# haoyu94/RoITr

Measured on AMD Instinct MI355X. Metric: point-cloud pairs/s, higher is better.
Workload: dtype f32; 1 GPU; 3DMatch-sized synthetic pairs: 5000 pts/cloud src+tgt, fp32, 3DMatch test settings (P=256 patches x 64 pts, 100 Sinkhorn iterations), full RIGA_v2 forward; n_points=5000, weights=closed-form, variant 'selective' (roitr_amd/weights.py); normals: field, cloud=uniform, correspondences_found=66241517

## Files before the change

### include/roitr_engine.h

```cpp
#ifndef ROITR_ENGINE_H
#define ROITR_ENGINE_H

#include <stddef.h>

#ifdef __cplusplus
extern "C" {
#endif

#ifndef ROITR_POINTOPS_H
typedef struct ihipStream_t* roitr_stream_t;
#endif

typedef struct RoitrGemm {
    int M, N, K;
    const float* A; const float* A2; int lda; const int* a_idx; int a_limit;
    const float* W; int ldw; const int* w_idx; int w_limit;
    const float* bias; float alpha; int relu;
    float* C; int ldc;
    int batch; long sA, sW, sC, sBias, sAidx, sWidx;
    const int* seg_off; int seg_a0, seg_w0;
    const float* ln_gamma; const float* ln_beta; const float* ln_res; const int* ln_res_idx; const float* ln_post;
    int ln_relu; float ln_eps;
    int bf16;
    const float* A_cat; int lda_cat; int k_cat;
    const float* ip_feat; const int* ip_idx; const float* ip_dist2;
    const int* a_cat_idx;
    const int* batch_live;
    long w_piece;
} RoitrGemm;
#define ROITR_BF16_W 1
#define ROITR_BF16_A 2
#define ROITR_BF16_C 4
#define ROITR_BF16_X3 8
int roitr_gemm(const RoitrGemm* g, roitr_stream_t stream);
int roitr_gemm_bf16_supported(const RoitrGemm* g);
int roitr_f32_to_bf16(long n, const float* src, unsigned short* dst, roitr_stream_t stream);
int roitr_gemm_x3_supported(const RoitrGemm* g);
int roitr_split_bf16x3(long n, const float* src, unsigned short* dst, long piece, roitr_stream_t stream);

int roitr_add_layernorm(int M, int C, const float* x, const float* res, const int* res_idx, const float* gamma,
                        const float* beta, const float* post_add, int relu, float eps, float* out, roitr_stream_t stream);
int roitr_add_layernorm_interp(int M, int C, const float* x, const float* res, const int* res_idx, const float* gamma,
                               const float* beta, int relu, float eps, const float* ip_feat, const int* ip_idx, const float* ip_dist2,
                               float* out, roitr_stream_t stream);
int roitr_l2_normalize(int M, int C, const float* x, float* out, roitr_stream_t stream);
int roitr_transpose(int rows, int cols, const float* in, int ld_in, float* out, int ld_out, roitr_stream_t stream);
int roitr_add_vectors(int n, const float* a, const float* b, float* out, roitr_stream_t stream);
int roitr_interp3_add(int n, int C, const float* feat, const int* idx, const float* dist2, const float* base, float* out,
                      roitr_stream_t stream);
int roitr_segment_mean(int b, int C, const float* x, const int* offset, float* out, roitr_stream_t stream);
int roitr_sinusoid(long rows, int C, const float* vals, const float* div_term, float* out, roitr_stream_t stream);
int roitr_geo_embed(long rows, int C, int angle_k, const float* d_idx, const float* a_idx, const float* div_term,
                    const float* Wd, const float* bd, const float* Wa, const float* ba, float* out, roitr_stream_t stream);
int roitr_split3_bf16(long n, const float* src, unsigned short* dst, roitr_stream_t stream);
int roitr_geo_embed_split(long rows, int C, int angle_k, const float* d_idx, const float* a_idx, const float* div_term,
                          const unsigned short* Wd3, const float* bd, const unsigned short* Wa3, const float* ba, float* out,
                          roitr_stream_t stream);
int roitr_geo_embed_bf16(long rows, int C, int angle_k, const float* d_idx, const float* a_idx, const float* div_term,
                         const unsigned short* Wd, const float* bd, const unsigned short* Wa, const float* ba, float* out,
                         roitr_stream_t stream);
int roitr_geo_embed_bf16_out(long rows, int C, int angle_k, const float* d_idx, const float* a_idx, const float* div_term,
                             const unsigned short* Wd, const float* bd, const unsigned short* Wa, const float* ba,
                             unsigned short* out, roitr_stream_t stream);
size_t roitr_geo_table_floats(int C, int n_int_d, int n_int_a);
int roitr_geo_table_build(int C, const float* div_term, const float* Wd, const float* bd, const float* Wa, const float* ba,
                          float interval, int n_int_d, int n_int_a, float* table, double* fit);
int roitr_geo_embed_table(long rows, int C, int angle_k, const float* d_idx, const float* a_idx, const float* table, float interval,
                          int n_int_d, int n_int_a, const float* div_term, const float* Wd, const float* bd, const float* Wa,
                          const float* ba, void* out, int out_bf16, roitr_stream_t stream);
int roitr_geo_combine(long rows, int C, int k, const float* pd, const float* pa, float* out, roitr_stream_t stream);
int roitr_gather_rows(long rows, int C, const float* in, const int* idx, int limit, float* out, roitr_stream_t stream);
int roitr_compose_idx(int n, const int* outer, const int* inner, int* out, roitr_stream_t stream);
int roitr_calc_ppf(int m, int k, const float* centre_xyz, const float* centre_normals, const float* ref_xyz,
                   const float* ref_normals, const int* group_idx, float* out, roitr_stream_t stream);

typedef struct RoitrLocalAttn {
    int M, K, H, heads;
    const float* q; int ldq;
    const float* k; int ldk;
    const float* v; int ldv;
    const int* group_idx; const float* ppf;
    const float* wvpe; const float* bvpe;
    float scale;
    float* out; int ldo;
    const void* node_order;
    int bf16;
    const float* wpe; const float* bpe;
} RoitrLocalAttn;
// ... 154 lines not shown
    int num_corr;
    int point_limit;
    int fine_topk, fine_mutual, fine_use_global_score;
    float fine_conf;
    int n_geo_layers;
    int geo_is_cross[16];
    float matching_radius;
    int adaptive_coarse;
    float occlusion_radius;
    int operand_dtype;
} RoitrEngineConfig;

typedef struct RoitrForwardIO {
    int pairs;
    const int* n_points;
    const float* points_geom;
    const float* normals;
    const float* feats;
    const float* points_out;
    const float* rot;
    const float* trans;
    float* node_xyz;
    float* node_feats;
    float* point_feats;
    int* node_masks;
    int* node_knn_idx;
    int* node_knn_mask;
    int* tgt_corr; int* src_corr; float* corr_scores; int* n_corr;
    float* tgt_knn_pts; float* src_knn_pts;
    int* tgt_knn_masks; int* src_knn_masks;
    float* matching_scores;
    float* out_tgt_pts; float* out_src_pts; float* out_scores; int* out_patch;
    int* fine_offsets;
    int* n_out;
    float* gt_node_occ;
    int* gt_corr_idx;
    float* gt_corr_overlaps;
    int* gt_corr_count;
    void* inputs_ready;
    int* patch_offsets;
    int* pair_starts;
    int patch_slots;
} RoitrForwardIO;

void* roitr_engine_create(const RoitrEngineConfig* cfg);
void roitr_engine_destroy(void* engine);
int roitr_engine_set_param(void* engine, const char* name, const float* device_ptr, long numel);
int roitr_engine_finalize(void* engine, roitr_stream_t stream);
int roitr_engine_geo_table_info(void* engine, double* info);
int roitr_engine_forward(void* engine, const RoitrForwardIO* io, roitr_stream_t stream);
int roitr_engine_forward_graph(void* engine, const RoitrForwardIO* io, roitr_stream_t stream);
int roitr_engine_graph_count(void* engine);
int roitr_engine_set_phase_overlap(void* engine, int on);
int roitr_engine_scratch_info(void* engine, long* out5);
int roitr_engine_set_tap(void* engine, const char* name, void* device_ptr);
int roitr_engine_set_inject(void* engine, const char* name, const void* device_ptr);
void roitr_level_sizes(int n, int* out4);


int roitr_inlier_counts(int pairs, const int* starts, const float* src_pts, const float* tgt_pts, const float* rot,
                        const float* trans, float radius, int* inliers, roitr_stream_t stream);
int roitr_coarse_hits(int pairs, int num_corr, const int* n_corr, const int* tgt_corr, const int* src_corr, int gt_cap,
                      const int* gt_idx, const float* gt_overlaps, const int* gt_count, float acceptance_overlap, int* hits,
                      roitr_stream_t stream);


size_t roitr_registration_workspace_bytes(int pairs, int total_rows, int iterations, int chunks);
int roitr_ransac_correspondences(int pairs, const int* starts, int total_rows, const float* src_pts, const float* tgt_pts,
                                 const float* scores, const unsigned int* pair_keys, int sample_mode, int n_points, int ransac_n,
                                 float distance_threshold, float edge_similarity, int iterations, int refine_iters, int refine_weighted,
                                 unsigned long long seed, int chunks, void* workspace, size_t workspace_bytes, float* transforms,
                                 int* inliers, int* best_iteration, int* valid_hypotheses, int* n_used, int* selected,
                                 roitr_stream_t stream);
int roitr_ransac_samples(int pairs, const int* n, const unsigned int* pair_keys, unsigned long long seed, int it0, int count, int* out,
                         roitr_stream_t stream);
int roitr_weighted_procrustes(int batch, int n, const float* src_pts, const float* tgt_pts, const float* weights, float weight_thresh,
                              float eps, float* transforms, roitr_stream_t stream);


#define ROITR_LGR_NO_ROWS 1
#define ROITR_LGR_NO_LOCAL 2
#define ROITR_LGR_EMPTY_REFIT 4
size_t roitr_lgr_workspace_bytes(int pairs, int total_rows);
int roitr_lgr_batch(int pairs, const int* starts, int total_rows, const float* src_pts, const float* tgt_pts, const float* scores,
                    const int* row_patch, float radius, int min_rows, int steps, void* workspace, size_t workspace_bytes,
                    float* transforms, int* inliers, int* best_hypothesis, int* best_first_row, int* hypotheses, int* local_inliers,
                    int* status, int* hyp_starts, int* hyp_first_row, float* hyp_transforms, int* hyp_counts, roitr_stream_t stream);


#define ROITR_COMPAT_NO_ROWS 1
#define ROITR_COMPAT_NO_HYPOTHESIS 2
#define ROITR_COMPAT_EMPTY_REFIT 4
#define ROITR_COMPAT_TRUNCATED 8
size_t roitr_compat_workspace_bytes(int pairs, int total_rows, int max_rows, int max_seeds, int k);
int roitr_compat_batch(int pairs, const int* starts, int total_rows, const float* src_pts, const float* tgt_pts, const float* scores,
                       float compat_dist, float radius, int max_rows, int max_seeds, int k, int steps, void* workspace,
                       size_t workspace_bytes, float* transforms, int* inliers, int* best_rank, int* best_seed_row, int* seeds,
                       int* hypotheses, int* local_inliers, int* status, int* degree, int* seed_rows, int* seed_members,
                       float* hyp_transforms, int* hyp_counts, roitr_stream_t stream);


#define ROITR_NFMR_FEW_ANCHORS 1
#define ROITR_NFMR_NO_METRIC 2
#define ROITR_NFMR_BAD_INDEX 4
#define ROITR_NFMR_BAD_OFFSETS 8
size_t roitr_nfmr_workspace_bytes(int pairs, int total_corr, int total_metric);
// ... 39 lines not shown
```

### roitr_amd/csrc/engine.cpp

```cpp
#include <hip/hip_runtime.h>
#include <math.h>
#include <stdio.h>
#include <string.h>

#include <map>
#include <string>
#include <vector>

#include "common.h"
#include "prof.h"
#include "roitr_engine.h"
#include "roitr_pointops.h"

#define CHK(x)                    \
    do {                          \
        int s__ = (x);            \
        if (s__ != 0) return s__; \
    } while (0)

namespace {

constexpr int HEADS = 4;
constexpr int GRID_MIN_POINTS = 768;

struct Lin {
    const float* w = nullptr; const float* b = nullptr; int out = 0, in = 0;
    const unsigned short* wb = nullptr;
};

struct LocalT {
    Lin emb, in_proj, q, k, v, p, vp, lin, out_proj;
    const float* norm_w = nullptr; const float* norm_b = nullptr;
    int in_dim = 0, H = 0, out_dim = 0;
    float* wqkv = nullptr;
    unsigned short* wqkv_b = nullptr;
    float* bqkv = nullptr;
    float* wqkv_x = nullptr; float* bqkv_x = nullptr; unsigned short* wqkv_x_b = nullptr;
    float* wkT_x = nullptr;
    float* wqqt_x = nullptr; float* bqqt_x = nullptr;
    float* wcat = nullptr; float* bcat = nullptr; unsigned short* wcat_b = nullptr;
    const float* wpe = nullptr; const float* bpe = nullptr;
    float* wvpe = nullptr;
    float* bvpe = nullptr;
    const float* bn2_w = nullptr; const float* bn2_b = nullptr;
};

struct Up {
    Lin l1, l2; const float* l1n_w = nullptr; const float* l1n_b = nullptr; const float* l2n_w = nullptr; const float* l2n_b = nullptr;
};

struct Ffn {
    Lin expand, squeeze; const float* n_w = nullptr; const float* n_b = nullptr;
};

struct GeoLayer {
    bool cross = false;
    Lin q, k, v, p, vp, lin, pos_lin;
    const float *n_w = nullptr, *n_b = nullptr, *pn_w = nullptr, *pn_b = nullptr;
    Ffn out, pos;
    float* wqkv = nullptr; float* bqkv = nullptr;
    float* wpT = nullptr;
    unsigned short* wqkv_b = nullptr; unsigned short* wpT_b = nullptr;
};

struct Arena {
    char* base = nullptr; size_t cap = 0, off = 0, peak = 0;
    bool fail = false;
    template <typename T> T* get(size_t count)
    {
        const size_t bytes = (count * sizeof(T) + 255) & ~(size_t)255;
        if (off + bytes > cap) { fail = true; return (T*)base; }
        T* p = base ? (T*)(base + off) : nullptr;
        off += bytes;
        if (off > peak) peak = off;
        return p;
    }
};

struct Engine {
    RoitrEngineConfig cfg;
    std::map<std::string, std::pair<const float*, long>> params;
    std::map<std::string, void*> taps;
    std::map<std::string, const void*> injects;
    bool finalized = false;
    int planes[4];
    int nblocks[4] = {2, 3, 3, 3};
    int nsample[4] = {8, 16, 16, 16};
    LocalT enc[4][3];
    LocalT dec[4];
    Up up[4];
    Lin geo_in, geo_out, proj_d, proj_a, coarse_proj, fine_proj;
    const float* geo_div = nullptr;
    float* geo_div_own = nullptr;
    float* geo_tab = nullptr; float geo_tab_h = 0.f; int geo_tab_nd = 0, geo_tab_na = 0; double geo_tab_fit[6] = {0, 0, 0, 0, 0, 0};
    std::vector<GeoLayer> geo;
    const float* ot_alpha = nullptr;
    float* first_consts = nullptr;
    Arena warena;
    Arena arena;
    Arena barena;
    Arena garena[2];
    int gpar = 0;
    int cur_par = -1;
    hipEvent_t gend[2] = {nullptr, nullptr};
    bool gend_rec[2] = {false, false};
    bool ahead_off = false;
    bool garena_short = false;
    static constexpr int RING = 4;
    char* pinned[RING] = {nullptr, nullptr, nullptr, nullptr}; size_t pinned_cap[RING] = {0, 0, 0, 0};
    hipEvent_t pinned_ev[RING] = {nullptr, nullptr, nullptr, nullptr};
    int ring_pos = 0;
    hipStream_t side = nullptr;
    enum Ev {
        EV_MAIN_BEGIN,
        EV_LEVEL2_GEOM_DONE,
        EV_LEVEL3_GEOM_DONE,
        EV_LEVEL4_GEOM_DONE,
        EV_LEVEL1_WS_FREE,
        EV_EMBED_DONE,
        EV_NN3_DONE,
        EV_TAIL_DONE,
        EV_ERROR_JOIN,
        EV_DESC_COPIED,
        EV_LEVEL1_GROUPS_READY,
        EV_ENCODER_DONE,
        EV_BRANCH_DONE,
        EV_BRANCH_ERROR_JOIN,
        NEV
    };
    static Ev ev_level_done(int l) { return (Ev)(EV_LEVEL2_GEOM_DONE + l - 1); }
    hipEvent_t ev[NEV] = {};
    bool side_forked = false;
    hipStream_t branch = nullptr;
    int phase_overlap = 1;
    bool branch_forked = false;
    bool on_branch = false;
    std::string err;
    hipStream_t fin_stream = nullptr;
    struct GraphEntry {
        std::vector<long> key;
        hipGraph_t graph = nullptr; hipGraphExec_t exec = nullptr;
        char* pin = nullptr; size_t pin_cap = 0;
        long epoch = -1;
        bool warmed = false, failed = false;
        unsigned long stamp = 0;
    };
    std::vector<GraphEntry> graphs;
    long arena_epoch = 0;
    unsigned long graph_clock = 0;
    char* capture_pin = nullptr;
    std::map<std::pair<const float*, long>, unsigned short*> x3;
    std::vector<const float*> frag_weights;
};

thread_local Engine* g_engine = nullptr;

int use_x3(RoitrGemm& g, hipStream_t st)
{
    Engine* E = g_engine;
    if (!E || E->cfg.operand_dtype != 2 || !E->finalized || g.bf16 || g.K < 256 || g.ldw != g.K || g.batch != 1 || g.ln_gamma) return 0;
    RoitrGemm t = g;
    t.bf16 = ROITR_BF16_X3; t.w_piece = (long)g.N * g.K;
    const long numel = (long)g.N * g.K;
    const auto key = std::make_pair(g.W, numel);
    auto it = E->x3.find(key);
    unsigned short* w3 = nullptr;
    if (it != E->x3.end()) w3 = it->second;
    else {
        if (E->capture_pin) return 0;
        if (hipMalloc((void**)&w3, sizeof(unsigned short) * 3 * (size_t)numel) != hipSuccess) { (void)hipGetLastError(); return 0; }
        if (roitr_split_bf16x3(numel, g.W, w3, numel, st) != ROITR_OK) { (void)hipFree(w3); return 0; }
        E->x3[key] = w3;
    }
    t.W = reinterpret_cast<const float*>(w3);
    if (!roitr_gemm_x3_supported(&t)) return 0;
    g = t;
    return 0;
}

const float* P(Engine& E, const std::string& name, long expect)
{
    auto it = E.params.find(name);
    if (it == E.params.end()) { if (E.err.empty()) E.err = "missing parameter " + name; return nullptr; }
    if (expect > 0 && it->second.second != expect) {
        if (E.err.empty()) E.err = "parameter " + name + " has " + std::to_string(it->second.second) + " elements, expected " + std::to_string(expect);
        return nullptr;
    }
    return it->second.first;
}

Lin lin(Engine& E, const std::string& prefix, int out, int in)
{
    Lin l;
    l.w = P(E, prefix + ".weight", (long)out * in);
    l.b = P(E, prefix + ".bias", out);
    l.out = out; l.in = in;
    if (E.cfg.operand_dtype == 1 && l.w) {
        unsigned short* wb = E.warena.get<unsigned short>((size_t)out * in);
        if (!E.warena.fail && roitr_f32_to_bf16((long)out * in, l.w, wb, E.fin_stream) == 0) l.wb = wb;
    }
    return l;
}

bool bf16_layer(const unsigned short* Wb, int K) { return Wb != nullptr && K % 64 == 0; }
int use_bf16(RoitrGemm& g, const float* W, const unsigned short* Wb, int bf)
{
    if (Wb) {
        g.W = reinterpret_cast<const float*>(Wb);
        g.bf16 = ROITR_BF16_W | bf;
        if (roitr_gemm_bf16_supported(&g)) return 0;
        g.W = W; g.bf16 = 0;
    }
    if (bf) { roitr_set_error("engine: bf16-stored activation routed to an fp32 layer", __FILE__, __LINE__); return ROITR_ERR_ARG; }
    return 0;
}
int gemm(hipStream_t st, int M, int N, int K, const float* A, int lda, const float* W, int ldw, const float* bias, float* C, int ldc,
         bool relu = false, const int* a_idx = nullptr, const float* A2 = nullptr, float alpha = 1.0f, const unsigned short* Wb = nullptr,
         int bf = 0)
{
    RoitrGemm g;
    memset(&g, 0, sizeof(g));
    g.M = M; g.N = N; g.K = K; g.A = A; g.A2 = A2; g.lda = lda; g.a_idx = a_idx; g.W = W; g.ldw = ldw; g.bias = bias;
    g.alpha = alpha; g.relu = relu ? 1 : 0; g.C = C; g.ldc = ldc; g.batch = 1;
    CHK(use_bf16(g, W, Wb, bf));
    CHK(use_x3(g, st));
    return roitr_gemm(&g, st);
}
int gemm(hipStream_t st, int M, const float* A, const Lin& l, float* C, bool relu = false, const int* a_idx = nullptr, const float* A2 = nullptr,
         int bf = 0)
{
    return gemm(st, M, l.out, l.in, A, l.in, l.w, l.in, l.b, C, l.out, relu, a_idx, A2, 1.0f, l.wb, bf);
}

struct Interp3 { const float* feat; const int* idx; const float* dist2; };
bool ln_fuses(int N, int K, int lda, int ldw)
{
    return (N == 64 || N == 128) && K % 32 == 0 && lda % 4 == 0 && ldw % 4 == 0;
}
int gemm_ln(hipStream_t st, int M, const float* A, const Lin& l, const float* res, const int* res_idx, const float* gamma,
            const float* beta, const float* post, bool relu, float* tmp, float* out, int bf = 0, const float* A_cat = nullptr,
            int lda_cat = 0, int k_cat = 0, const float* A2 = nullptr, const Interp3* ip = nullptr, const int* a_cat_idx = nullptr)
{
    const float* w = l.w;
    const float* b = l.b;
    const int K = l.in, N = l.out;
    const int lda = A_cat ? k_cat : K, ldw = K;
    if (ln_fuses(N, K, lda, ldw)) {
        RoitrGemm g;
        memset(&g, 0, sizeof(g));
        g.M = M; g.N = N; g.K = K; g.A = A; g.lda = lda; g.W = w; g.ldw = ldw; g.bias = b; g.alpha = 1.0f; g.C = out; g.ldc = N; g.batch = 1;
        g.ln_gamma = gamma; g.ln_beta = beta; g.ln_res = res; g.ln_res_idx = res_idx; g.ln_post = post; g.ln_relu = relu ? 1 : 0; g.ln_eps = 1e-5f;
        g.A_cat = A_cat; g.lda_cat = lda_cat; g.k_cat = k_cat; g.A2 = A2;
        g.a_cat_idx = a_cat_idx;
        if (ip) { g.ip_feat = ip->feat; g.ip_idx = ip->idx; g.ip_dist2 = ip->dist2; }
        CHK(use_bf16(g, w, l.wb, bf));
        return roitr_gemm(&g, st);
    }
    if (bf & ROITR_BF16_C) { roitr_set_error("engine: bf16 LayerNorm output needs the fused epilogue", __FILE__, __LINE__); return ROITR_ERR_ARG; }
    if (A_cat) {
        RoitrGemm g;
        memset(&g, 0, sizeof(g));
        g.M = M; g.N = N; g.K = K; g.A = A; g.lda = lda; g.W = w; g.ldw = ldw; g.bias = b; g.alpha = 1.0f; g.C = tmp; g.ldc = N; g.batch = 1;
        g.A_cat = A_cat; g.lda_cat = lda_cat; g.k_cat = k_cat; g.A2 = A2; g.a_cat_idx = a_cat_idx;
        CHK(use_x3(g, st));
        CHK(roitr_gemm(&g, st));
    } else
    CHK(gemm(st, M, N, K, A, lda, w, ldw, b, tmp, N, false, nullptr, A2, 1.0f, l.wb, bf));
    if (ip) {
        if (post) { roitr_set_error("engine: interpolation addend and post-add together", __FILE__, __LINE__); return ROITR_ERR_ARG; }
        return roitr_add_layernorm_interp(M, N, tmp, res, res_idx, gamma, beta, relu ? 1 : 0, 1e-5f, ip->feat, ip->idx, ip->dist2, out, st);
    }
    return roitr_add_layernorm(M, N, tmp, res, res_idx, gamma, beta, post, relu ? 1 : 0, 1e-5f, out, st);
}

int d2d(hipStream_t st, void* dst, const void* src, size_t bytes)
{
    ROITR_HIP(hipMemcpyAsync(dst, src, bytes, hipMemcpyDeviceToDevice, st));
    return 0;
}

int tap(Engine& E, hipStream_t st, const std::string& name, void* data, size_t bytes)
{
    auto ij = E.injects.find(name);
    if (ij != E.injects.end() && ij->second) CHK(d2d(st, data, ij->second, bytes));
    auto it = E.taps.find(name);
    if (it != E.taps.end() && it->second) CHK(d2d(st, it->second, data, bytes));
    return 0;
}

int resolve_local(Engine& E, LocalT& L, const std::string& pre, int in_dim, int H, int out_dim)
{
    L.in_dim = in_dim; L.H = H; L.out_dim = out_dim;
    L.emb = lin(E, pre + ".embedding.proj", H, 4);
    L.in_proj = lin(E, pre + ".in_proj", H, in_dim);
    const std::string at = pre + ".transformer.attention";
    L.q = lin(E, at + ".proj_q", H, H); L.k = lin(E, at + ".proj_k", H, H); L.v = lin(E, at + ".proj_v", H, H);
    L.p = lin(E, at + ".proj_p", H, H); L.vp = lin(E, at + ".proj_vp", H, H);
    L.lin = lin(E, pre + ".transformer.linear", H, H);
    L.norm_w = P(E, pre + ".transformer.norm.weight", H); L.norm_b = P(E, pre + ".transformer.norm.bias", H);
    L.out_proj = lin(E, pre + ".out_proj", out_dim, H);
// ... 1375 lines not shown
        fm.out_row_pts = o_t; fm.out_col_pts = o_s; fm.out_scores = o_sc; fm.out_patch = io->out_patch; fm.out_cap = (long)cap;
        fm.pair_off = pair_off; fm.slots = compact ? (int)NP : 0; fm.pair_starts = io->pair_starts;
        CHK(roitr_matching_tail(&o, &fm, st));
    }
    return 0;
}
}

static int forward_body(Engine& E, const RoitrForwardIO* io, hipStream_t st)
{
    if (!E.finalized) { roitr_set_error("engine not finalized", __FILE__, __LINE__); return ROITR_ERR_ARG; }
    if (io->pairs <= 0) return 0;
    Plan P; GeoBufs S; Feats F; BranchBufs R;
    P.st = st;
    CHK(plan_sizes(E, io, P));
    CHK(reserve_arenas(E, io, P));
    CHK(carve_geometry_buffers(E, io, P, S));
    carve_branch(io, P, E.barena, R);
    if (E.barena.fail) { roitr_set_error("arena exhausted (branch)", __FILE__, __LINE__); return ROITR_ERR_ARG; }
    CHK(stage_descriptors(E, P, S));
    hipStream_t sb = P.sb;
    roitr_prof_begin(ROITR_PROF_PH_FORWARD, 0.0, st);
    CHK(issue_geometry_chain(E, io, P, S));
    roitr_prof_begin(ROITR_PROF_PH_ENC, 0.0, st);   CHK(encoder(E, io, P, S, F));             roitr_prof_end(ROITR_PROF_PH_ENC, st);
    if (sb != st) {
        ROITR_HIP(hipEventRecord(E.ev[Engine::EV_ENCODER_DONE], st));
        ROITR_HIP(hipStreamWaitEvent(sb, E.ev[Engine::EV_ENCODER_DONE], 0));
        E.branch_forked = true;
    }
    const bool forked = sb != st;
    E.on_branch = forked;
    roitr_prof_begin(ROITR_PROF_PH_GEO, 0.0, sb);
    CHK(global_transformer(E, P, S, F, R));
    if (forked) CHK(coarse_front(E, P, S, F, R));
    roitr_prof_end(ROITR_PROF_PH_GEO, sb);
    if (forked) ROITR_HIP(hipEventRecord(E.ev[Engine::EV_BRANCH_DONE], sb));
    roitr_prof_begin(ROITR_PROF_PH_DEC, 0.0, st);   CHK(decoder(E, P, S, F));                 roitr_prof_end(ROITR_PROF_PH_DEC, st);
    roitr_prof_begin(ROITR_PROF_PH_MATCH, 0.0, st);
    if (!forked) CHK(coarse_front(E, P, S, F, R));
    CHK(heads_and_matching(E, io, P, F, R));
    roitr_prof_end(ROITR_PROF_PH_MATCH, st);
    roitr_prof_end(ROITR_PROF_PH_FORWARD, st);
    return 0;
}

extern "C" int roitr_engine_scratch_info(void* h, long* out5)
{
    Engine& E = *(Engine*)h;
    out5[0] = (long)E.arena.cap; out5[1] = (long)E.arena.peak; out5[2] = (long)E.barena.cap; out5[3] = (long)E.barena.peak;
    out5[4] = E.on_branch ? 1 : 0;
    return ROITR_OK;
}

extern "C" int roitr_engine_set_phase_overlap(void* h, int on)
{
    Engine& E = *(Engine*)h;
    const int mode = on == 0 ? 0 : on == 2 ? 2 : 1;
    if (E.phase_overlap != mode) { E.phase_overlap = mode; E.arena_epoch++; }
    return ROITR_OK;
}


extern "C" int roitr_engine_forward_graph(void* h, const RoitrForwardIO* io, hipStream_t st)
{
    Engine& E = *(Engine*)h;
    if (!E.finalized) { roitr_set_error("engine not finalized", __FILE__, __LINE__); return ROITR_ERR_ARG; }
    if (!st || roitr_prof_is_enabled() || !E.taps.empty() || !E.injects.empty() || io->pairs <= 0) return roitr_engine_forward(h, io, st);
    std::vector<long> key;
    key.push_back(io->pairs);
    long t4 = 0;
    for (int c = 0; c < 2 * io->pairs; ++c) { key.push_back(io->n_points[c]); int s4[4]; roitr_level_sizes(io->n_points[c], s4); t4 += s4[3]; }
    {
        const void* const* pp = reinterpret_cast<const void* const*>(&io->points_geom);
        const size_t n_ptr = (reinterpret_cast<const char*>(&io->patch_slots) - reinterpret_cast<const char*>(&io->points_geom)) / sizeof(void*);
        for (size_t i = 0; i < n_ptr; ++i) key.push_back((long)(uintptr_t)pp[i]);
        key.push_back(io->patch_slots);
    }
    Engine::GraphEntry* ge = nullptr;
    for (auto& g : E.graphs) if (g.key == key) { ge = &g; break; }
    if (!ge) {
        if (E.graphs.size() >= 16) {
            size_t lru = 0;
            for (size_t i = 1; i < E.graphs.size(); ++i) if (E.graphs[i].stamp < E.graphs[lru].stamp) lru = i;
            auto& g = E.graphs[lru];
            if (g.exec) (void)hipGraphExecDestroy(g.exec);
            if (g.graph) (void)hipGraphDestroy(g.graph);
            if (g.pin) (void)hipHostFree(g.pin);
            E.graphs.erase(E.graphs.begin() + lru);
        }
        E.graphs.emplace_back();
        ge = &E.graphs.back();
        ge->key = key;
    }
    ge->stamp = ++E.graph_clock;
    if (ge->failed) return roitr_engine_forward(h, io, st);
    if (!ge->warmed || ge->epoch != E.arena_epoch) {
        if (ge->exec) { (void)hipGraphExecDestroy(ge->exec); ge->exec = nullptr; }
        if (ge->graph) { (void)hipGraphDestroy(ge->graph); ge->graph = nullptr; }
        const int rc = roitr_engine_forward(h, io, st);
        ge->warmed = rc == ROITR_OK;
        ge->epoch = E.arena_epoch;
        return rc;
    }
    if (!ge->exec) {
        const size_t need = Desc::bytes(2 * (size_t)io->pairs, (size_t)t4) + 64;
        if (need > ge->pin_cap) {
// ... 35 lines not shown
```

### roitr_amd/csrc/gemm.hip

```cpp
#include "common.h"
#include <cstdio>
#include <cstdlib>
#include <map>
#include <string>
#include "gemm_host.h"
#include "gemm_tile.h"

namespace {

constexpr int BK = 32, LDR = 20;

__device__ __forceinline__ void load8(const float* __restrict__ p, int k, int K, bool vec_ok, float (&v)[8])
{
    if (p == nullptr) {
#pragma unroll
        for (int i = 0; i < 8; ++i) v[i] = 0.f;
        return;
    }
    if (vec_ok && k + 8 <= K) {
        const float4 a = *reinterpret_cast<const float4*>(p + k);
        const float4 b = *reinterpret_cast<const float4*>(p + k + 4);
        v[0] = a.x; v[1] = a.y; v[2] = a.z; v[3] = a.w; v[4] = b.x; v[5] = b.y; v[6] = b.z; v[7] = b.w;
    } else {
#pragma unroll
// ... 439 lines not shown
        for (int s = 0; s < 8; ++s) acc = __builtin_amdgcn_mfma_f32_16x16x4f32(af[s], bf[s], acc, 0, 0, 0);
        __builtin_amdgcn_sched_barrier(0);
    }
    const int col = n0 + wn * 16 + i;
    if (col < g.N) {
        const float bv = bias ? bias[col] : 0.f;
#pragma unroll
        for (int q = 0; q < 4; ++q) {
            const int row = m0 + wm * 16 + 4 * gq + q;
            if (row < g.M) {
                float x = acc[q] * g.alpha + bv;
                if (g.relu) x = fmaxf(x, 0.f);
                C[(size_t)row * g.ldc + col] = x;
            }
        }
    }
}

}

namespace {
struct ShapeStat { double ms = 0; long n = 0; };
struct ShapeLog {
    std::map<std::string, ShapeStat> m;
    ~ShapeLog() {
        for (auto& kv : m) fprintf(stderr, "GEMMSHAPE %s launches %ld ms %.4f\n", kv.first.c_str(), kv.second.n, kv.second.ms);
    }
};
struct ShapeTimer {
    const RoitrGemm* g; bool fast; hipStream_t stream;
    hipEvent_t e0 = nullptr, e1 = nullptr;
    ShapeTimer(const RoitrGemm* g_, bool fast_, hipStream_t st) : g(g_), fast(fast_), stream(st)
    {
        static const bool shapes = getenv("ROITR_GEMM_SHAPES") != nullptr;
        if (shapes) { (void)hipEventCreate(&e0); (void)hipEventCreate(&e1); (void)hipEventRecord(e0, stream); }
    }
    ~ShapeTimer()
    {
        if (!e0) return;
        (void)hipEventRecord(e1, stream); (void)hipEventSynchronize(e1);
        float ms = 0.f; (void)hipEventElapsedTime(&ms, e0, e1); (void)hipEventDestroy(e0); (void)hipEventDestroy(e1);
        static ShapeLog log;
        char key[160];
        snprintf(key, sizeof key, "M %d N %d K %d batch %d gather %d a2 %d relu %d seg %d fast %d ln %d bf16 %d", g->M, g->N, g->K, g->batch, g->a_idx != nullptr,
                 g->A2 != nullptr, g->relu, g->seg_off != nullptr, (int)fast, g->ln_gamma != nullptr, g->bf16);
        auto& st = log.m[key];
        st.ms += ms; st.n += 1;
    }
};
}

int roitr_gemm_bf16_launch(const RoitrGemm* g, hipStream_t stream);
int roitr_gemm_x3_launch(const RoitrGemm* g, hipStream_t stream);

extern "C" int roitr_gemm(const RoitrGemm* g, hipStream_t stream)
{
    if (g->M <= 0 || g->N <= 0 || g->batch <= 0) return ROITR_OK;
    if (g->K <= 0 || !g->A || !g->W || !g->C) { roitr_set_error("roitr_gemm: K <= 0 or a null operand", __FILE__, __LINE__); return ROITR_ERR_ARG; }
    auto al16 = [](const void* p, long stride_floats) { return ((uintptr_t)p & 15) == 0 && (stride_floats % 4) == 0; };
    if (g->bf16) {
        ShapeTimer timer(g, true, stream);
        return (g->bf16 & ROITR_BF16_X3) ? roitr_gemm_x3_launch(g, stream) : roitr_gemm_bf16_launch(g, stream);
    }
    const bool fast = g->K % BK == 0 && g->K <= ZERO_ROW_LEN && g->lda % 4 == 0 && g->ldw % 4 == 0 && al16(g->A, g->sA) && al16(g->W, g->sW) &&
                      (!g->A2 || al16(g->A2, g->sA));
    if (g->A_cat && (!fast || g->batch != 1 || g->seg_off || g->k_cat % BK || g->k_cat <= 0 || g->k_cat >= g->K || g->lda_cat % 4 ||
                     ((uintptr_t)g->A_cat & 15))) {
        roitr_set_error("roitr_gemm: K-concatenated A needs the fast path (K % 32, 16-byte rows), k_cat % 32 == 0, no batching", __FILE__, __LINE__);
        return ROITR_ERR_UNSUPPORTED;
    }
    if (g->a_cat_idx && !g->A_cat) { roitr_set_error("roitr_gemm: a_cat_idx without A_cat", __FILE__, __LINE__); return ROITR_ERR_ARG; }
    const bool ln = g->ln_gamma != nullptr;
    const int tn = ln ? g->N / BN : 1;
    if (ln && (!gemm_ln_shape_ok(g) || (!fast && tn != 1))) return ROITR_ERR_UNSUPPORTED;
    if (g->ip_feat && (!ln || !g->ip_idx || !g->ip_dist2)) { roitr_set_error("roitr_gemm: the interpolation addend rides in the fused LayerNorm epilogue only", __FILE__, __LINE__); return ROITR_ERR_UNSUPPORTED; }
    const int nx = div_up(g->N, BN * tn), ny = div_up(g->M, BM);
    int T;
    if (!gemm_tile_count(nx, ny, g->batch, &T)) return ROITR_ERR_UNSUPPORTED;
    const unsigned grid = (unsigned)xcd_grid(T);
    const int prof_cls = gemm_prof_begin(g, stream);
    {
    ShapeTimer timer(g, fast, stream);
    const bool a2 = g->A2 != nullptr;
    const bool il = T >= GEMM_IL_MIN_TILES;
    if (fast && !ln && T < GEMM_SMALL_MAX_TILES) {
        const int sx = div_up(g->N, SM), sy = div_up(g->M, SM);
        const int ST = sx * sy * g->batch;
        if (a2) gemm_small_kernel<true><<<xcd_grid(ST), 256, 0, stream>>>(*g, sx, sy, ST);
        else gemm_small_kernel<false><<<xcd_grid(ST), 256, 0, stream>>>(*g, sx, sy, ST);
    } else if (!fast) {
        if (ln) gemm_kernel<false, 1, true><<<grid, 256, 0, stream>>>(*g, nx, ny, T);
        else gemm_kernel<false, 1, false><<<grid, 256, 0, stream>>>(*g, nx, ny, T);
    } else
        dispatch_tn(tn, [&](auto tn_) {
            constexpr int TN = decltype(tn_)::value;
            auto launch = [&](auto ln_) {
                constexpr bool LN = decltype(ln_)::value;
                if (a2 && il) gemm_kernel<true, TN, LN, true, true><<<grid, 256, 0, stream>>>(*g, nx, ny, T);
                else if (a2) gemm_kernel<true, TN, LN, true, false><<<grid, 256, 0, stream>>>(*g, nx, ny, T);
                else if (il) gemm_kernel<true, TN, LN, false, true><<<grid, 256, 0, stream>>>(*g, nx, ny, T);
                else gemm_kernel<true, TN, LN, false, false><<<grid, 256, 0, stream>>>(*g, nx, ny, T);
            };
            if (ln) launch(std::true_type());
            else if constexpr (TN == 1) launch(std::false_type());
        });
    }
    roitr_prof_end(prof_cls, stream);
    ROITR_LAUNCH_CHECK();
    return ROITR_OK;
}
```

### roitr_amd/riga.py

```python
import ctypes
import math
import time

import numpy as np
import torch
import torch.nn as nn

from . import _args as A
from . import _lib as L


def _linear(prefix, out, inp):
    return [(prefix + ".weight", (out, inp), "param"), (prefix + ".bias", (out,), "param")]


def _norm(prefix, c):
    return [(prefix + ".weight", (c,), "param"), (prefix + ".bias", (c,), "param")]


def _local_transformer(prefix, inp, hidden, out):
    ent = [(prefix + ".embedding.embedding.div_term", (hidden // 2,), "buffer")]
    ent += _linear(prefix + ".embedding.proj", hidden, 4)
    ent += _linear(prefix + ".in_proj", hidden, inp)
    for n in ("proj_q", "proj_k", "proj_v", "proj_p", "proj_vp"):
# ... 180 lines not shown
        cfg.fine_topk = self.fine_topk
        cfg.fine_mutual = int(self.fine_mutual)
        cfg.fine_use_global_score = int(self.fine_use_global_score)
        cfg.fine_conf = self.fine_conf
        cfg.n_geo_layers = len(self.architecture)
        for i, a in enumerate(self.architecture):
            cfg.geo_is_cross[i] = 0 if a == "self" else 1
        cfg.matching_radius = self.matching_radius
        cfg.adaptive_coarse = 0 if self.factor == 1 else 1
        cfg.occlusion_radius = 0.0375
        cfg.operand_dtype = {"f32": 0, "bf16": 1, "f32x3": 2}[self.operand_dtype]
        lib.roitr_engine_create.restype = ctypes.c_void_p
        h = lib.roitr_engine_create(ctypes.byref(cfg))
        if not h:
            raise L.RoitrError("roitr_engine_create failed")
        return ctypes.c_void_p(h)

    def sync_engine(self):
        lib = L.lib()
        if self._engine is None:
            self._engine = self._make_engine()
        for k, v in self.state_dict(keep_vars=True).items():
            if not v.is_cuda:
                raise L.RoitrError(f"parameter {k} is not on a ROCm device: call model.cuda() (no CPU fallback)")
            if v.dtype != torch.float32 or not v.is_contiguous():
                raise L.RoitrError(f"parameter {k} must be contiguous float32")
            L.check(lib.roitr_engine_set_param(self._engine, k.encode(), L.ptr(v), ctypes.c_long(v.numel())), "set_param")
        L.check(lib.roitr_engine_finalize(self._engine, L.stream_ptr()), "engine_finalize")
        self._holders = list(self.modules())
        self._engine_sig = self._weights_signature()

    def _weights_signature(self):
        return [(t.data_ptr(), t._version) for m in self._holders for d in (m._parameters, m._buffers) for t in d.values() if t is not None]

    def _ensure_engine(self):
        if self._engine is None or (not self.weights_frozen and self._weights_signature() != self._engine_sig):
            self.sync_engine()

    def set_tap(self, name, tensor):
        self._ensure_engine()
        self._taps = getattr(self, "_taps", {})
        self._taps[name] = tensor
        L.lib().roitr_engine_set_tap(self._engine, name.encode(), L.ptr(tensor))

    def set_inject(self, name, tensor):
        self._ensure_engine()
        self._injects = getattr(self, "_injects", {})
        self._injects[name] = tensor
        L.lib().roitr_engine_set_inject(self._engine, name.encode(), L.ptr(tensor))

    def set_phase_overlap(self, on=1):
        self._ensure_engine()
        L.check(L.lib().roitr_engine_set_phase_overlap(self._engine, ctypes.c_int(int(on))), "set_phase_overlap")

    def scratch_info(self):
        self._ensure_engine()
        out = (ctypes.c_long * 5)()
        L.check(L.lib().roitr_engine_scratch_info(self._engine, out), "scratch_info")
        return {"main_cap": out[0], "main_peak": out[1], "branch_cap": out[2], "branch_fill": out[3], "on_branch_stream": bool(out[4])}

    PROF_CLASSES = {"fps_kernel": 0, "knn_query_kernel": 1, "grid_build_kernel": 2, "knn_replay_kernel": 3, "phase.geometry": 4,
                    "phase.encoder": 5, "phase.global_transformer": 6, "phase.decoder": 7, "phase.matching": 8,
                    "phase.forward": 9, "ot_kernel": 10, "local_attn_kernel": 11, "gemm_kernel.mfma_roofed": 12, "mha_kernel": 13,
                    "geo_embed_kernel": 14, "geo_table_kernel": 15, "geo_embed_reference_flops": 16, "local_block_kernel": 17,
                    "gemm_kernel.hbm_roofed": 18}

    @staticmethod
    def profile_reset(enable=True):
        lib = L.lib()
        lib.roitr_prof_enable(1 if enable else 0)
        lib.roitr_prof_reset()

    @classmethod
    def profile_read(cls, kernels_only=True):
        lib = L.lib()
        out = {}
        for name, cid in cls.PROF_CLASSES.items():
            ms, n, by = ctypes.c_double(0), ctypes.c_long(0), ctypes.c_double(0)
            lib.roitr_prof_read(cid, ctypes.byref(ms), ctypes.byref(n), ctypes.byref(by))
            aux = ctypes.c_double(0)
            lib.roitr_prof_read_aux(cid, ctypes.byref(aux))
            if n.value and (not kernels_only or not name.startswith("phase.")):
                out[name] = {"ms": ms.value, "launches": n.value, "bytes": by.value, "aux": aux.value}
        parts = [out[k] for k in ("gemm_kernel.mfma_roofed", "gemm_kernel.hbm_roofed") if k in out]
        if parts:
            out["gemm_kernel"] = {f: sum(p[f] for p in parts) for f in ("ms", "launches", "bytes", "aux")}
        lib.roitr_prof_enable(0)
        return out

    def geo_table_info(self):
        self._ensure_engine()
        info = (ctypes.c_double * 9)()
        if not L.lib().roitr_engine_geo_table_info(self._engine, info):
            return None
        keys = ("interval", "n_int_d", "n_int_a", "fit_d", "amp_d", "fit_a", "amp_a", "rel_d", "rel_a")
        out = dict(zip(keys, list(info)))
        out["lds_bytes"] = int((out["n_int_d"] + out["n_int_a"]) * 8 * 64 * 4)
        return out

    def __del__(self):
        try:
            if self._engine is not None:
                L.lib().roitr_engine_destroy(self._engine)
        except Exception:
            pass

# ... 279 lines not shown
```

Measured before the change: 6457 pairs/s.

## Add fused GEMM+LayerNorm kernel for 256-wide outputs on large row counts

Adds a dedicated MFMA GEMM kernel with N=256 that parks the 32-row output tile in LDS and applies bias, residual add, LayerNorm, optional post-add, ReLU and 3-NN interpolation in its epilogue. gemm_ln routes eligible calls (N=256, K<=512, fp32 operands, rows above a threshold, no in-place gathered residual) to it instead of a separate GEMM plus add-layernorm pass. The aim is to avoid writing the intermediate to memory and the extra launch. In exchange, each block covers only 32 rows, which may reduce MFMA efficiency. The row threshold can be tuned from Python.

```diff
diff --git a/include/roitr_engine.h b/include/roitr_engine.h
--- a/include/roitr_engine.h
+++ b/include/roitr_engine.h
@@ -34,6 +34,7 @@
 #define ROITR_BF16_X3 8
 int roitr_gemm(const RoitrGemm* g, roitr_stream_t stream);
 int roitr_gemm_bf16_supported(const RoitrGemm* g);
+int roitr_gemm_set_ln256_tile(int rows);
 int roitr_f32_to_bf16(long n, const float* src, unsigned short* dst, roitr_stream_t stream);
 int roitr_gemm_x3_supported(const RoitrGemm* g);
 int roitr_split_bf16x3(long n, const float* src, unsigned short* dst, long piece, roitr_stream_t stream);
@@ -294,6 +295,7 @@
 int roitr_engine_forward_graph(void* engine, const RoitrForwardIO* io, roitr_stream_t stream);
 int roitr_engine_graph_count(void* engine);
 int roitr_engine_set_phase_overlap(void* engine, int on);
+int roitr_engine_set_ln256_min_rows(void* engine, int rows);
 int roitr_engine_scratch_info(void* engine, long* out5);
 int roitr_engine_set_tap(void* engine, const char* name, void* device_ptr);
 int roitr_engine_set_inject(void* engine, const char* name, const void* device_ptr);
diff --git a/roitr_amd/csrc/engine.cpp b/roitr_amd/csrc/engine.cpp
--- a/roitr_amd/csrc/engine.cpp
+++ b/roitr_amd/csrc/engine.cpp
@@ -76,6 +76,10 @@
         return p;
     }
 };
+
+constexpr int LN256_MIN_ROWS = 39936;
+constexpr int LN256_MAX_K = 512;
+constexpr int LN256_NEVER = 0x7fffffff;
 
 struct Engine {
     RoitrEngineConfig cfg;
@@ -133,6 +137,7 @@
     bool side_forked = false;
     hipStream_t branch = nullptr;
     int phase_overlap = 1;
+    int ln256_min_rows = LN256_MIN_ROWS;
     bool branch_forked = false;
     bool on_branch = false;
     std::string err;
@@ -237,6 +242,12 @@
 {
     return (N == 64 || N == 128) && K % 32 == 0 && lda % 4 == 0 && ldw % 4 == 0;
 }
+bool ln256_fuses(int M, int N, int K, int lda, int ldw, const Lin& l, int bf)
+{
+    const Engine* E = g_engine;
+    if (!E || E->cfg.operand_dtype != 0 || l.wb || bf) return false;
+    return N == 256 && K % 32 == 0 && K <= LN256_MAX_K && lda % 4 == 0 && ldw % 4 == 0 && M >= E->ln256_min_rows;
+}
 int gemm_ln(hipStream_t st, int M, const float* A, const Lin& l, const float* res, const int* res_idx, const float* gamma,
             const float* beta, const float* post, bool relu, float* tmp, float* out, int bf = 0, const float* A_cat = nullptr,
             int lda_cat = 0, int k_cat = 0, const float* A2 = nullptr, const Interp3* ip = nullptr, const int* a_cat_idx = nullptr)
@@ -245,7 +256,8 @@
     const float* b = l.b;
     const int K = l.in, N = l.out;
     const int lda = A_cat ? k_cat : K, ldw = K;
-    if (ln_fuses(N, K, lda, ldw)) {
+    const bool gather_in_place = res_idx && res == out;
+    if (ln_fuses(N, K, lda, ldw) || (ln256_fuses(M, N, K, lda, ldw, l, bf) && !gather_in_place)) {
         RoitrGemm g;
         memset(&g, 0, sizeof(g));
         g.M = M; g.N = N; g.K = K; g.A = A; g.lda = lda; g.W = w; g.ldw = ldw; g.bias = b; g.alpha = 1.0f; g.C = out; g.ldc = N; g.batch = 1;
@@ -1727,6 +1739,14 @@
     return ROITR_OK;
 }
 
+extern "C" int roitr_engine_set_ln256_min_rows(void* h, int rows)
+{
+    Engine& E = *(Engine*)h;
+    const int r = rows < 0 ? LN256_MIN_ROWS : rows == 0 ? LN256_NEVER : rows;
+    if (E.ln256_min_rows != r) { E.ln256_min_rows = r; E.arena_epoch++; }
+    return ROITR_OK;
+}
+
 extern "C" int roitr_engine_set_phase_overlap(void* h, int on)
 {
     Engine& E = *(Engine*)h;
diff --git a/roitr_amd/csrc/gemm.hip b/roitr_amd/csrc/gemm.hip
--- a/roitr_amd/csrc/gemm.hip
+++ b/roitr_amd/csrc/gemm.hip
@@ -515,6 +515,8 @@
 
 int roitr_gemm_bf16_launch(const RoitrGemm* g, hipStream_t stream);
 int roitr_gemm_x3_launch(const RoitrGemm* g, hipStream_t stream);
+bool roitr_gemm_ln256_takes(const RoitrGemm* g);
+void roitr_gemm_ln256_launch(const RoitrGemm* g, hipStream_t stream);
 
 extern "C" int roitr_gemm(const RoitrGemm* g, hipStream_t stream)
 {
@@ -546,7 +548,9 @@
     ShapeTimer timer(g, fast, stream);
     const bool a2 = g->A2 != nullptr;
     const bool il = T >= GEMM_IL_MIN_TILES;
-    if (fast && !ln && T < GEMM_SMALL_MAX_TILES) {
+    if (fast && ln && tn == 4 && roitr_gemm_ln256_takes(g)) {
+        roitr_gemm_ln256_launch(g, stream);
+    } else if (fast && !ln && T < GEMM_SMALL_MAX_TILES) {
         const int sx = div_up(g->N, SM), sy = div_up(g->M, SM);
         const int ST = sx * sy * g->batch;
         if (a2) gemm_small_kernel<true><<<xcd_grid(ST), 256, 0, stream>>>(*g, sx, sy, ST);
diff --git a/roitr_amd/csrc/gemm_ln256.hip b/roitr_amd/csrc/gemm_ln256.hip
--- /dev/null
+++ b/roitr_amd/csrc/gemm_ln256.hip
@@ -0,0 +1,259 @@
+#include "common.h"
+#include "gemm_host.h"
+#include "gemm_tile.h"
+
+namespace {
+
+constexpr int BK = 32, LDR = 20;
+constexpr int LM = 32, LC = 256;
+constexpr int LN256_IL_MIN_TILES = 1024;
+constexpr int LN256_ZERO_LEN = 2048;
+__device__ __attribute__((aligned(16))) float g_ln256_zero_row[LN256_ZERO_LEN];
+
+template <bool HA2, bool IL>
+__global__ __launch_bounds__(256) void gemm_ln256_kernel(RoitrGemm g, int T)
+{
+    constexpr int STAGE = 2 * LM * LDR + 2 * LC * LDR, TP = LC + 1;
+    static_assert(LM * TP <= STAGE, "the parked tile must fit the staging LDS");
+    __shared__ __attribute__((aligned(16))) float smem[STAGE];
+    float* As = smem;
+    float* Bs = smem + 2 * LM * LDR;
+    const int tile = xcd_block_id_live(T);
+    if (tile < 0) return;
+    const int m0 = tile * LM;
+    const float* bias = g.bias;
+    float* C = g.C;
+
+    const int tid = threadIdx.x, lane = tid & 63, wave = tid >> 6;
+    const int r = tid >> 2, kq = (tid & 3) * 8, kf = (tid & 3) * 4;
+    const int ra = tid >> 3, ja = tid & 3, ha = (tid >> 2) & 1, ka = 4 * ja + 16 * ha;
+
+    const float* arow = g_ln256_zero_row; const float* arow2 = g_ln256_zero_row; const float* arowc = g_ln256_zero_row;
+    {
+        const int am = m0 + ra;
+        if (am < g.M) {
+            arow = g.A + (size_t)am * g.lda;
+            if (HA2) arow2 = g.A2 + (size_t)am * g.lda;
+            if (g.A_cat) arowc = g.A_cat + (size_t)(g.a_cat_idx ? g.a_cat_idx[am] : am) * g.lda_cat;
+        }
+    }
+    const float* wrow[4];
+#pragma unroll
+    for (int v = 0; v < 4; ++v) wrow[v] = g.W + (size_t)(r + 64 * v) * g.ldw + kf;
+
+    f32x16 acc[2];
+#pragma unroll
+    for (int v = 0; v < 2; ++v)
+#pragma unroll
+        for (int i = 0; i < 16; ++i) acc[v][i] = 0.f;
+
+    float4 av, a2v = make_float4(0.f, 0.f, 0.f, 0.f);
+    float wv[4][8];
+    auto asrc = [&](int k) { return ((g.A_cat && k >= g.k_cat) ? arowc + (k - g.k_cat) : arow + k) + ka; };
+    auto a2src = [&](int k) { return ((g.A_cat && k >= g.k_cat) ? g_ln256_zero_row : arow2 + k) + ka; };
+    {
+        av = *reinterpret_cast<const float4*>(asrc(0));
+        if (HA2) a2v = *reinterpret_cast<const float4*>(a2src(0));
+#pragma unroll
+        for (int v = 0; v < 4; ++v) {
+            const float4 x = *reinterpret_cast<const float4*>(wrow[v]), y = *reinterpret_cast<const float4*>(wrow[v] + 16);
+            wv[v][0] = x.x; wv[v][1] = x.y; wv[v][2] = x.z; wv[v][3] = x.w; wv[v][4] = y.x; wv[v][5] = y.y; wv[v][6] = y.z; wv[v][7] = y.w;
+        }
+    }
+    const int kh = lane >> 5, ml = lane & 31;
+    const float4* ar = reinterpret_cast<const float4*>(As + (kh * LM + ml) * LDR);
+    const float4* br = reinterpret_cast<const float4*>(Bs + (kh * LC + wave * 64 + ml) * LDR);
+    float2* aw0 = reinterpret_cast<float2*>(As + (0 * LM + ra) * LDR + 4 * ja + 2 * ha);
+    float2* aw1 = reinterpret_cast<float2*>(As + (1 * LM + ra) * LDR + 4 * ja + 2 * ha);
+    float4* bw0 = reinterpret_cast<float4*>(Bs + (0 * LC + r) * LDR + (kq >> 1));
+    float4* bw1 = reinterpret_cast<float4*>(Bs + (1 * LC + r) * LDR + (kq >> 1));
+    for (int k0 = 0; k0 < g.K; k0 += BK) {
+        __syncthreads();
+        if (HA2) { av.x += a2v.x; av.y += a2v.y; av.z += a2v.z; av.w += a2v.w; }
+        *aw0 = make_float2(av.x, av.z); *aw1 = make_float2(av.y, av.w);
+#pragma unroll
+        for (int v = 0; v < 4; ++v) {
+            bw0[v * 64 * LDR / 4] = make_float4(wv[v][0], wv[v][2], wv[v][4], wv[v][6]);
+            bw1[v * 64 * LDR / 4] = make_float4(wv[v][1], wv[v][3], wv[v][5], wv[v][7]);
+        }
+        __syncthreads();
+        float4 af[4], bf[2][4];
+        if (!IL) {
+            if (k0 + BK < g.K) {
+                const int kn = k0 + BK;
+                av = *reinterpret_cast<const float4*>(asrc(kn));
+                if (HA2) a2v = *reinterpret_cast<const float4*>(a2src(kn));
+#pragma unroll
+                for (int v = 0; v < 4; ++v) {
+                    const float4 x = *reinterpret_cast<const float4*>(wrow[v] + kn), y = *reinterpret_cast<const float4*>(wrow[v] + kn + 16);
+                    wv[v][0] = x.x; wv[v][1] = x.y; wv[v][2] = x.z; wv[v][3] = x.w; wv[v][4] = y.x; wv[v][5] = y.y; wv[v][6] = y.z; wv[v][7] = y.w;
+                }
+            }
+        }
+#pragma unroll
+        for (int q = 0; q < 4; ++q) {
+            af[q] = ar[q];
+#pragma unroll
+            for (int v = 0; v < 2; ++v) bf[v][q] = br[v * 32 * LDR / 4 + q];
+        }
+        __builtin_amdgcn_sched_barrier(0);
+        const int kn = k0 + BK < g.K ? k0 + BK : k0;
+        const float* an = asrc(kn);
+        const float* a2n = a2src(kn);
+        constexpr int NS = 1 + (HA2 ? 1 : 0) + 8, TOT = 32;
+#pragma unroll
+        for (int q = 0; q < 4; ++q)
+#pragma unroll
+            for (int c = 0; c < 4; ++c)
+#pragma unroll
+                for (int v = 0; v < 2; ++v) {
+                    const float a = c == 0 ? af[q].x : c == 1 ? af[q].y : c == 2 ? af[q].z : af[q].w;
+                    const float b = c == 0 ? bf[v][q].x : c == 1 ? bf[v][q].y : c == 2 ? bf[v][q].z : bf[v][q].w;
+                    acc[v] = __builtin_amdgcn_mfma_f32_32x32x2f32(a, b, acc[v], 0, 0, 0);
+                    if (IL) {
+                        const int n = (q * 4 + c) * 2 + v;
+#pragma unroll
+                        for (int i = 0; i < NS; ++i)
+                            if (n == (i * TOT + TOT / 2) / NS) {
+                                __builtin_amdgcn_sched_barrier(0);
+                                if (i == 0) av = *reinterpret_cast<const float4*>(an);
+                                else if (HA2 && i == 1) a2v = *reinterpret_cast<const float4*>(a2n);
+                                else {
+                                    const int j = i - 1 - (HA2 ? 1 : 0), h = j & 1, wr = j >> 1;
+                                    const float4 x = *reinterpret_cast<const float4*>(wrow[wr] + kn + 16 * h);
+                                    wv[wr][4 * h] = x.x; wv[wr][4 * h + 1] = x.y; wv[wr][4 * h + 2] = x.z; wv[wr][4 * h + 3] = x.w;
+                                }
+                                __builtin_amdgcn_sched_barrier(0);
+                            }
+                    }
+                }
+        __builtin_amdgcn_sched_barrier(0);
+    }
+
+    float gam[4], bet[4];
+#pragma unroll
+    for (int i = 0; i < 4; ++i) { gam[i] = g.ln_gamma[lane + 64 * i]; bet[i] = g.ln_beta[lane + 64 * i]; }
+    float resv[8][4], postv[8][4];
+#pragma unroll
+    for (int u = 0; u < 8; ++u) {
+        const int row_ = m0 + wave + 4 * u;
+#pragma unroll
+        for (int i = 0; i < 4; ++i) { resv[u][i] = 0.f; postv[u][i] = 0.f; }
+        if (row_ < g.M) {
+            if (g.ln_res) {
+                const float* rr = g.ln_res + (size_t)(g.ln_res_idx ? g.ln_res_idx[row_] : row_) * LC;
+#pragma unroll
+                for (int i = 0; i < 4; ++i) resv[u][i] = rr[lane + 64 * i];
+            }
+            if (g.ln_post) {
+#pragma unroll
+                for (int i = 0; i < 4; ++i) postv[u][i] = g.ln_post[(size_t)row_ * LC + lane + 64 * i];
+            }
+        }
+    }
+    float* tile_ = smem;
+    __syncthreads();
+#pragma unroll
+    for (int v = 0; v < 2; ++v) {
+        const int col = wave * 64 + v * 32 + (lane & 31);
+        const float bv = bias ? bias[col] : 0.f;
+#pragma unroll
+        for (int i = 0; i < 16; ++i) {
+            const int rl = (i & 3) + 8 * (i >> 2) + 4 * (lane >> 5);
+            tile_[rl * TP + col] = acc[v][i] * g.alpha + bv;
+        }
+    }
+    __syncthreads();
+    int pi0 = 0, pi1 = 0, pi2 = 0; float pw0 = 0.f, pw1 = 0.f, pw2 = 0.f;
+    float fn0[4], fn1[4], fn2[4];
+    if (g.ip_feat) {
+        const int rowl = m0 + wave + 4 * lane;
+        if (lane < LM / 4 && rowl < g.M) {
+            const int* ii = g.ip_idx + (size_t)rowl * 3;
+            const float* dd = g.ip_dist2 + (size_t)rowl * 3;
+            pi0 = ii[0]; pi1 = ii[1]; pi2 = ii[2];
+            pw0 = 1.0f / (sqrtf(dd[0]) + 1e-8f); pw1 = 1.0f / (sqrtf(dd[1]) + 1e-8f); pw2 = 1.0f / (sqrtf(dd[2]) + 1e-8f);
+            const float ws = (pw0 + pw1) + pw2;
+            pw0 /= ws; pw1 /= ws; pw2 /= ws;
+        }
+        const float* a0 = g.ip_feat + (size_t)__builtin_amdgcn_readlane(pi0, 0) * LC;
+        const float* a1 = g.ip_feat + (size_t)__builtin_amdgcn_readlane(pi1, 0) * LC;
+        const float* a2 = g.ip_feat + (size_t)__builtin_amdgcn_readlane(pi2, 0) * LC;
+#pragma unroll
+        for (int i = 0; i < 4; ++i) { fn0[i] = a0[lane + 64 * i]; fn1[i] = a1[lane + 64 * i]; fn2[i] = a2[lane + 64 * i]; }
+    }
+#pragma unroll
+    for (int u = 0; u < 8; ++u) {
+        const int rl = wave + 4 * u;
+        const int row = m0 + rl;
+        if (row >= g.M) break;
+        float fc0[4], fc1[4], fc2[4];
+        float w0 = 0.f, w1 = 0.f, w2 = 0.f;
+        if (g.ip_feat) {
+#pragma unroll
+            for (int i = 0; i < 4; ++i) { fc0[i] = fn0[i]; fc1[i] = fn1[i]; fc2[i] = fn2[i]; }
+            w0 = __int_as_float(__builtin_amdgcn_readlane(__float_as_int(pw0), u));
+            w1 = __int_as_float(__builtin_amdgcn_readlane(__float_as_int(pw1), u));
+            w2 = __int_as_float(__builtin_amdgcn_readlane(__float_as_int(pw2), u));
+            if (u + 1 < 8 && row + 4 < g.M) {
+                const float* a0 = g.ip_feat + (size_t)__builtin_amdgcn_readlane(pi0, (u + 1) & 7) * LC;
+                const float* a1 = g.ip_feat + (size_t)__builtin_amdgcn_readlane(pi1, (u + 1) & 7) * LC;
+                const float* a2 = g.ip_feat + (size_t)__builtin_amdgcn_readlane(pi2, (u + 1) & 7) * LC;
+#pragma unroll
+                for (int i = 0; i < 4; ++i) { fn0[i] = a0[lane + 64 * i]; fn1[i] = a1[lane + 64 * i]; fn2[i] = a2[lane + 64 * i]; }
+            }
+        }
+        float t[4];
+        float s_ = 0.f;
+#pragma unroll
+        for (int i = 0; i < 4; ++i) {
+            t[i] = tile_[rl * TP + lane + 64 * i];
+            if (g.ln_res) t[i] += resv[u][i];
+            s_ += t[i];
+        }
+        const float mean = wave_sum(s_) / (float)LC;
+        float q_ = 0.f;
+#pragma unroll
+        for (int i = 0; i < 4; ++i) { const float d = t[i] - mean; q_ += d * d; }
+        const float rstd = 1.0f / sqrtf(wave_sum(q_) / (float)LC + g.ln_eps);
+#pragma unroll
+        for (int i = 0; i < 4; ++i) {
+            float y = (t[i] - mean) * rstd * gam[i] + bet[i];
+            if (g.ln_post) y += postv[u][i];
+            if (g.ln_relu) y = fmaxf(y, 0.f);
+            if (g.ip_feat) {
+                float acc_ = 0.f;
+                acc_ += fc0[i] * w0; acc_ += fc1[i] * w1; acc_ += fc2[i] * w2;
+                y = y + acc_;
+            }
+            C[(size_t)row * g.ldc + lane + 64 * i] = y;
+        }
+    }
+}
+
+int g_ln256_tile_rows = LM;
+
+}
+
+extern "C" int roitr_gemm_set_ln256_tile(int rows)
+{
+    g_ln256_tile_rows = rows == 64 ? 64 : LM;
+    return ROITR_OK;
+}
+
+bool roitr_gemm_ln256_takes(const RoitrGemm* g)
+{
+    return g_ln256_tile_rows == LM && g->ln_gamma && g->N == LC && !g->bf16 && !g->a_idx && !g->w_idx && g->a_limit <= 0 && g->w_limit <= 0 &&
+           g->batch == 1 && !g->seg_off && !g->batch_live && g->K <= LN256_ZERO_LEN && div_up(g->M, LM) <= 0x7ffffff0 / 8;
+}
+
+void roitr_gemm_ln256_launch(const RoitrGemm* g, hipStream_t stream)
+{
+    const int T = div_up(g->M, LM);
+    const unsigned grid = (unsigned)xcd_grid(T);
+    const bool a2 = g->A2 != nullptr, il = T >= LN256_IL_MIN_TILES;
+    if (a2 && il) gemm_ln256_kernel<true, true><<<grid, 256, 0, stream>>>(*g, T);
+    else if (a2) gemm_ln256_kernel<true, false><<<grid, 256, 0, stream>>>(*g, T);
+    else if (il) gemm_ln256_kernel<false, true><<<grid, 256, 0, stream>>>(*g, T);
+    else gemm_ln256_kernel<false, false><<<grid, 256, 0, stream>>>(*g, T);
+}
diff --git a/roitr_amd/riga.py b/roitr_amd/riga.py
--- a/roitr_amd/riga.py
+++ b/roitr_amd/riga.py
@@ -256,6 +256,10 @@
     def set_phase_overlap(self, on=1):
         self._ensure_engine()
         L.check(L.lib().roitr_engine_set_phase_overlap(self._engine, ctypes.c_int(int(on))), "set_phase_overlap")
+
+    def set_ln256_min_rows(self, rows=-1):
+        self._ensure_engine()
+        L.check(L.lib().roitr_engine_set_ln256_min_rows(self._engine, ctypes.c_int(int(rows))), "set_ln256_min_rows")
 
     def scratch_info(self):
         self._ensure_engine()
```

After: 6559 pairs/s, median of 6. 1.6% higher.
